# VladimirP1/rs-sync

Hardware: AMD Instinct MI355X
Metric: ray-residuals/sec (PreSync sweep + Sync iter), 4096 frames x 2048 tracks (higher is better)
Workload: dtype f32

## Files before the change

### rs-sync_amd/csrc/kernels/sync64.hpp

```cpp
#pragma once

#pragma clang fp contract(off)

namespace {



struct Loss64Params {
    Rays64 rays;
    const FrameRec* frames;
    const uint32_t* sel;
    uint32_t n_sel;
    const d4* coef;
    int n_knots;
    double fs;
    const int32_t* kd;
    const double* fd;
    uint32_t n_delays;
    const uint32_t* grp;
    uint32_t n_grp;
    const double* M;
    const double* k;
    double* part_loss;
    double* part_grad;
    uint32_t slot0;
    const uint32_t* slots;
    uint32_t win_cap;
    uint32_t win_compact;
    uint32_t nb_run;
};

constexpr int kLossBatch = 5;
constexpr int kLossBatchWide = 3;

template <int RPT, bool GRAD, bool SIMPLE, int CAP = 0>
__global__ __launch_bounds__(kBlock, 3) void loss64_kernel(Loss64Params p) {
    constexpr int NB = GRAD ? 1 : (CAP ? kLossBatch : (RPT == 0 ? 2 : kLossBatchWide));
    d4* s_loss_win;
    uint32_t win_cap;
    if constexpr (CAP != 0) {
        __shared__ d4 s_loss_win_static[NB * 4 * CAP];
        s_loss_win = s_loss_win_static;
        win_cap = CAP;
    } else {
        extern __shared__ d4 s_loss_win_dynamic[];
        s_loss_win = s_loss_win_dynamic;
        win_cap = p.win_cap;
    }
    __shared__ double s_red[NB][2][4];
    const uint32_t nb_run = (GRAD || CAP) ? (uint32_t)NB : (p.nb_run < (uint32_t)NB ? (p.nb_run ? p.nb_run : 1u) : (uint32_t)NB);
    const int tid = threadIdx.x, lane = tid & 63, wave = tid >> 6;
    const uint32_t sf = p.slots ? p.slots[blockIdx.x] : blockIdx.x + p.slot0;
    const uint32_t g = p.grp ? p.grp[sf] : 0u;
    {
        bool any = false;
        for (uint32_t b = 0; b < p.n_delays; ++b) {
            const double f = p.fd[b * p.n_grp + g];
            any = any || f == f;
        }
        if (!any) {
            for (uint32_t b = tid; b < p.n_delays; b += kBlock) {
                p.part_loss[(size_t)b * p.n_sel + sf] = 0.0;
                if (GRAD) p.part_grad[(size_t)b * p.n_sel + sf] = 0.0;
            }
            return;
        }
    }
    const uint32_t fi = p.sel[sf];
    const FrameRec fr = p.frames[fi];
    const uint32_t N = fr.n;
    const double Mx = SIMPLE ? 0.0 : p.M[3 * sf], My = SIMPLE ? 0.0 : p.M[3 * sf + 1], Mz = SIMPLE ? 0.0 : p.M[3 * sf + 2];
    const double kk = p.k[sf];
    const d3 Mv = d3{Mx, My, Mz};
    const double inv_s = rs::loss_inv_s(SIMPLE, kk, Mv);

    for (uint32_t b0 = 0; b0 < p.n_delays; b0 += nb_run) {
        Spline64 sp[NB];
        int base[NB];
        double fdv[NB];
        bool on[NB], any_on = false;
        int kdv[NB];
#pragma unroll
        for (int q = 0; q < NB; ++q) {
            const uint32_t b = b0 + q;
            on[q] = (uint32_t)q < nb_run && b < p.n_delays;
            kdv[q] = on[q] ? p.kd[b * p.n_grp + g] : 0;
            fdv[q] = on[q] ? p.fd[b * p.n_grp + g] : 0.0;
            if (fdv[q] != fdv[q]) on[q] = false;
            any_on = any_on || on[q];
        }
        if (!any_on) {
            if ((uint32_t)tid < nb_run && b0 + tid < p.n_delays) {
                p.part_loss[(size_t)(b0 + tid) * p.n_sel + sf] = 0.0;
                if (GRAD) p.part_grad[(size_t)(b0 + tid) * p.n_sel + sf] = 0.0;
            }
            continue;
        }
        __syncthreads();
// ... 144 lines not shown
    const int32_t* kd;
    const double* fd;
    const uint32_t* grp;
    double* M;
    double* k;
    unsigned long long* stats;
    uint32_t* per_frame;
    int reeval;
    int max_iters;
    int32_t* init_h;
    uint64_t seed;
    uint32_t stream_base, stream_stride;
    const uint32_t* win_stream;
    int simple_k;
    uint32_t slot0;
    const uint32_t* order;
    uint32_t* evals_out;
    double* scratch;
    uint32_t scratch_rows;
    uint32_t scratch0;
    uint32_t win_cap;
    uint32_t win_compact;
    uint32_t win_bytes;
};

#ifndef RSSYNC_K3_TIMING
#define RSSYNC_K3_TIMING 0
#endif
#if RSSYNC_K3_TIMING && RSSYNC_K2_COUNTERS
#define K3_T0() const long long k3t0__ = clock64()
#define K3_ACC(v) do { (v) += clock64() - k3t0__; } while (0)
#define K3_ADD(i, n) do { if (threadIdx.x == 0) { atomicAdd(&g_k2_counters[i], (unsigned long long)(clock64() - k3t0__)); if (n) atomicAdd(&g_k2_counters[n], 1ull); } } while (0)
#define K3_FLUSH(ev) do { if (threadIdx.x == 0) { atomicAdd(&g_k2_counters[10], (unsigned long long)(ev).t_eval); atomicAdd(&g_k2_counters[11], (unsigned long long)(ev).evals); } } while (0)
#else
#define K3_T0() do { } while (0)
#define K3_ACC(v) do { } while (0)
#define K3_ADD(i, n) do { } while (0)
#define K3_FLUSH(ev) do { } while (0)
#endif

constexpr int kInitNone = (int)0x80000000;
constexpr int kNB = rs::kLbfgsBasis;

template <int RPT, int NW, bool EMU4 = false>
struct MotionEval64 {
    static_assert(!EMU4 || (RPT == 0 && NW == 1), "the emulation reads its rows from global memory, one wave");
// ... 85 lines not shown
    __device__ __forceinline__ double& alpha(int i) { return s_alpha[i]; }
    __device__ __forceinline__ void store(int op, const double sv[3], const double yv[3]) {
        __syncthreads();
        if (threadIdx.x == 0) {
            for (int c = 0; c < 3; ++c) { s_S[op][c] = sv[c]; s_Y[op][c] = yv[c]; }
            s_inv_ys[op] = 1.0 / rs::dot3(yv, sv);
        }
        __syncthreads();
    }
};

__device__ __forceinline__ double clamp_k(double k) { return rs::clamp_k64(k); }

template <int NW>
struct MotionLds {
    double part[2][NW][4];
    double S[kNB][3], Y[kNB][3];
    double rho[kNB], alpha[kNB];
    double inv_ys[kNB];
    double red[NW];
};

template <int RPT, int NW, bool SC1 = false, bool EMU4 = false>
__device__ __forceinline__ void opt_motion64_body(const Motion64Params& p, uint32_t sf, MotionLds<NW>& lds, d4* s_win, double* mk_out = nullptr,
                                                  uint32_t scratch_entry = 0) {
    constexpr int kThreads = 64 * NW;
    double (*s_part)[NW][4] = lds.part;
    double (*s_S)[3] = lds.S;
    double (*s_Y)[3] = lds.Y;
    double* s_rho = lds.rho;
    double* s_alpha = lds.alpha;
    double* s_inv_ys = lds.inv_ys;
    double* s_red = lds.red;
    const int tid = threadIdx.x;
    const uint32_t fi = p.sel[sf];
    const FrameRec fr = p.frames[fi];
    const uint32_t N = fr.n;
    const uint32_t grp = p.grp ? p.grp[sf] : 0u;
    const int kd = ld_m<SC1>(&p.kd[grp]);
    const double fd = ld_m<SC1>(&p.fd[grp]);
    const int pend = p.init_h ? ld_m<SC1>(&p.init_h[sf]) : kInitNone;
    const double m_x = ld_m<SC1>(&p.M[3 * sf]), m_y = ld_m<SC1>(&p.M[3 * sf + 1]), m_z = ld_m<SC1>(&p.M[3 * sf + 2]);
    const double m_k = ld_m<SC1>(&p.k[sf]);
    if (fd != fd) {
        if (tid == 0 && p.evals_out) p.evals_out[sf] = 0;
        if (mk_out) { mk_out[0] = m_x; mk_out[1] = m_y; mk_out[2] = m_z; mk_out[3] = m_k; }
        return;
    }

    Spline64 sp;
    sp.g = p.coef;
    sp.n = p.n_knots;
    sp.cap = (int)p.win_cap;
    sp.compact = (int)p.win_compact;
    frame_window64(sp, s_win, fr, kd);
    __syncthreads();

    MotionEval64<RPT, NW, EMU4> ev;
    ev.part = s_part;
    ev.buf = 0;
    ev.evals = 0;
    const int base = fr.base_knot + kd;
    ev.gP = nullptr;
    ev.g_rows = 0;
    ev.rpt = RPT;
    if constexpr (RPT != 0) {
// ... 60 lines not shown
                const double pm = p.simple_k ? sqrt(rs::dot(Pj, Pj)) : rs::dot(Pj, Mv);
                ss = fma(pm, pm, ss);
            }
        }
        const double sw = wave_sum_f64(ss);
        if ((tid & 63) == 0) s_red[tid >> 6] = sw;
        __syncthreads();
        tot = s_red[0];
#pragma unroll
        for (int w = 1; w < NW; ++w) tot += s_red[w];
        }
        kk = clamp_k(100.0 / sqrt(tot));
        x[0] = Mv.x; x[1] = Mv.y; x[2] = Mv.z;
        if (tid == 0) {
            if (!p.simple_k) { st_m<SC1>(&p.M[3 * sf], x[0]); st_m<SC1>(&p.M[3 * sf + 1], x[1]); st_m<SC1>(&p.M[3 * sf + 2], x[2]); }
            st_m<SC1>(&p.k[sf], kk);
            if (p.init_h) st_m<SC1>(&p.init_h[sf], (int32_t)kInitNone);
        }
    } else {
        x[0] = m_x; x[1] = m_y; x[2] = m_z;
        kk = m_k;
    }
    if (mk_out) { mk_out[0] = x[0]; mk_out[1] = x[1]; mk_out[2] = x[2]; mk_out[3] = kk; }
    if (p.max_iters <= 0 || p.simple_k) return;
    ev.k2 = kk * kk;
    if constexpr (EMU4) {
        if ((size_t)N * 24u <= (size_t)p.win_bytes) {
            __syncthreads();
            __attribute__((address_space(3))) double* l = (__attribute__((address_space(3))) double*)reinterpret_cast<double*>(s_win);
            for (uint32_t row = tid; row < N; row += kThreads) {
                l[row] = ev.gP[row];
                l[N + row] = ev.gP[ev.g_rows + row];
                l[2 * N + row] = ev.gP[2 * (size_t)ev.g_rows + row];
            }
            __syncthreads();
            ev.lP = l;
            ev.n_lds = N;
        }
    }

    LbfgsHistLds hist{s_S, s_Y, s_inv_ys, s_rho, s_alpha};
    int best_not_last = 0;
    K3_T0();
    const int it = rs::lbfgs3(ev, hist, x, p.max_iters , p.reeval, &best_not_last);
    K3_ADD(12, 13);
    K3_FLUSH(ev);
    if (mk_out) { mk_out[0] = x[0]; mk_out[1] = x[1]; mk_out[2] = x[2]; }
    if (tid == 0) {
        st_m<SC1>(&p.M[3 * sf], x[0]); st_m<SC1>(&p.M[3 * sf + 1], x[1]); st_m<SC1>(&p.M[3 * sf + 2], x[2]);
        if (p.stats) {
            atomicAdd(&p.stats[0], (unsigned long long)it);
            atomicAdd(&p.stats[1], (unsigned long long)ev.evals);
            atomicAdd(&p.stats[2], (unsigned long long)best_not_last);
        }
        if (p.per_frame) {
            p.per_frame[2 * sf] = (uint32_t)it;
            p.per_frame[2 * sf + 1] = (uint32_t)ev.evals;
        }
        if (p.evals_out) p.evals_out[sf] = (uint32_t)ev.evals;
    }
}

template <int RPT, int NW>
__global__ __launch_bounds__(64 * NW, NW == 4 ? (RPT == 0 ? 2 : (RPT <= 8 ? 3 : (RPT <= 24 ? 2 : 1))) : (NW == 1 ? (RPT >= 8 ? 3 : 4) : 2)) void opt_motion64_kernel(Motion64Params p) {
    __shared__ MotionLds<NW> lds;
    extern __shared__ d4 s_motion_win[];
    opt_motion64_body<RPT, NW>(p, p.order ? p.order[blockIdx.x + p.slot0] : blockIdx.x + p.slot0, lds, s_motion_win, nullptr,
                               p.scratch0 + blockIdx.x);
}

__global__ __launch_bounds__(1024) void motion_order_kernel(const uint32_t* __restrict__ evals, const uint32_t* __restrict__ list,
                                                            uint32_t* __restrict__ order, uint32_t pos0, uint32_t count) {
    __shared__ uint32_t s_bin[256];
    for (uint32_t b = threadIdx.x; b < 256; b += blockDim.x) s_bin[b] = 0;
    __syncthreads();
    for (uint32_t i = threadIdx.x; i < count; i += blockDim.x) {
        const uint32_t e = evals[list[pos0 + i]];
        atomicAdd(&s_bin[e < 255u ? e : 255u], 1u);
    }
    __syncthreads();
    if (threadIdx.x == 0) {
        uint32_t at = 0;
        for (int b = 255; b >= 0; --b) {
            const uint32_t n = s_bin[b];
            s_bin[b] = at;
            at += n;
        }
    }
    __syncthreads();
    for (uint32_t i = threadIdx.x; i < count; i += blockDim.x) {
        const uint32_t s = list[pos0 + i];
        const uint32_t e = evals[s];
        const uint32_t pos = atomicAdd(&s_bin[e < 255u ? e : 255u], 1u);
        order[pos0 + pos] = s;
    }
}

struct Debug64Params {
    Rays64 rays;
    const FrameRec* frames;
    uint32_t fi;
    const d4* coef;
    int n_knots;
    double fs;
    int32_t kd;
    double fd;
    double* P;
    double* dP;
};

__global__ __launch_bounds__(kBlock) void debug_problem64_kernel(Debug64Params p) {
    __shared__ d4 s_win[4 * kWinMax];
    const FrameRec fr = p.frames[p.fi];
    Spline64 sp;
    sp.g = p.coef;
    sp.n = p.n_knots;
    sp.cap = kWinMax;
    sp.compact = 0;
// ... 31 lines not shown
```

### rs-sync_amd/csrc/kernels/syncloop.hpp

```cpp
#pragma once

namespace {

constexpr int kMaxBt = 10, kHalfBt = 5;

struct SyncWin {
    double d, v;
    double x0;
    double l1, g1;
    int active, conv, hit, iters;
    int phase;
    int nf;
    int hit_prev;
};

struct SyncLoopParams {
    SyncWin* win;
    uint32_t n_win;
    uint32_t win0, win1;
    const double* part;
    uint32_t n_sel, rows;
    const uint32_t* chunk_off;
    const uint32_t* win_chunk_off;
    double* chunk_tmp;
    uint32_t chunk_stride;
    int32_t* mo_kd; double* mo_fd;
    int32_t* lg_kd; double* lg_fd;
    int32_t* tr_kd; double* tr_fd;
    double fs;
    double ts[11];
    double c_armijo, delay_b, search_center, search_radius;
    int it, max_outer;
    int nf_fixed;
    int nf_floor;
    double* ext_sums;
    int* n_active;
    double* trace;
};


__device__ __forceinline__ void split64_dev(double delay, double fs, int32_t* kd, double* fd) {
#pragma clang fp contract(off)
    if (delay != delay) { *kd = 0; *fd = delay; return; }
    const double D = delay * fs;
    const double kClamp = (double)(1 << 29);
    if (!(fabs(D) <= 1.79769313486231570e308)) { *kd = 0; *fd = 0.0; return; }
    const double fl = floor(D);
    if (fl > kClamp) { *kd = 1 << 29; *fd = 0.0; return; }
    if (fl < -kClamp) { *kd = -(1 << 29); *fd = 0.0; return; }
    *kd = (int32_t)fl;
    *fd = D - fl;
}

constexpr uint32_t kStageDoubles = 2048;
__device__ __forceinline__ void window_sums(const SyncLoopParams& p, uint32_t w, double* s_tot, double* s_stage) {
    const uint32_t c0 = p.win_chunk_off[w], c1 = p.win_chunk_off[w + 1], nc = c1 - c0;
    const uint32_t j_lo = p.chunk_off[c0], j_hi = p.chunk_off[c1], span = j_hi - j_lo;
    double* tmp = p.chunk_tmp + (size_t)w * (2 * kMaxBt) * p.chunk_stride;
    const bool staged = p.rows * span <= kStageDoubles;
    if (staged) {
        for (uint32_t e = threadIdx.x; e < p.rows * span; e += blockDim.x)
            s_stage[e] = p.part[(size_t)(e / span) * p.n_sel + j_lo + e % span];
        __syncthreads();
    }
    for (uint32_t e = threadIdx.x; e < p.rows * nc; e += blockDim.x) {
        const uint32_t r = e / nc, c = c0 + e % nc;
        double acc = 0.0;
        uint32_t j = p.chunk_off[c];
        const uint32_t j1 = p.chunk_off[c + 1];
        if (staged) {
            const double* row = s_stage + (size_t)r * span - j_lo;
            for (; j + 8 <= j1; j += 8) {
                double v[8];
#pragma unroll
                for (int q = 0; q < 8; ++q) v[q] = row[j + q];
#pragma unroll
                for (int q = 0; q < 8; ++q) acc += v[q];
            }
            for (; j < j1; ++j) acc += row[j];
        } else {
            const double* row = p.part + (size_t)r * p.n_sel;
            const uint32_t cnt = j1 - j;
            if (cnt <= 64) {
                double v[64];
#pragma unroll
                for (int q = 0; q < 64; ++q) v[q] = (uint32_t)q < cnt ? row[j + q] : 0.0;
#pragma unroll
                for (int q = 0; q < 64; ++q)
                    if ((uint32_t)q < cnt) acc += v[q];
            } else {
                for (; j < j1; ++j) acc += row[j];
            }
        }
        tmp[(size_t)r * p.chunk_stride + (c - c0)] = acc;
    }
    __syncthreads();
    for (uint32_t r = threadIdx.x; r < p.rows; r += blockDim.x) {
        const double* t = tmp + (size_t)r * p.chunk_stride;
        double acc = 0.0;
        uint32_t c = 0;
        for (; c + 16 <= nc; c += 16) {
            double v[16];
#pragma unroll
            for (int q = 0; q < 16; ++q) v[q] = t[c + q];
#pragma unroll
            for (int q = 0; q < 16; ++q) acc += v[q];
        }
        for (; c < nc; ++c) acc += t[c];
        s_tot[r] = acc;
    }
    __syncthreads();
}

__global__ __launch_bounds__(64) void sync_begin_kernel(SyncLoopParams p) {
#pragma clang fp contract(off)
    const uint32_t w = p.win0 + blockIdx.x * 64 + threadIdx.x;
    if (w >= p.win1) return;
    SyncWin& s = p.win[w];
    s.x0 = s.active ? s.d - p.delay_b * s.v : __builtin_nan("");
    split64_dev(s.active ? s.d : __builtin_nan(""), p.fs, &p.mo_kd[w], &p.mo_fd[w]);
    split64_dev(s.x0, p.fs, &p.lg_kd[w], &p.lg_fd[w]);
}

__device__ __forceinline__ bool trial_wanted(const SyncWin& s, int i) {
    if (!s.active) return false;
    return s.phase == 0 ? i < s.nf : i >= s.nf;
}

__device__ __forceinline__ void grad_decide(const SyncLoopParams& p, SyncWin& s, double l1, double g1) {
#pragma clang fp contract(off)
    if (s.active && s.phase == 0) {
        s.l1 = l1;
        s.g1 = g1;
        s.hit = -1;
        if (s.iters == 0 && !p.nf_fixed) {
            int i = 0;
            while (i < kMaxBt - 1 && p.ts[i] * fabs(s.g1) >= 1e-3) ++i;
            const int want = i + 2;
            s.nf = want < kHalfBt ? kHalfBt : (want > kMaxBt ? kMaxBt : want);
        }
    }
}
__device__ __forceinline__ void trial_delays(const SyncLoopParams& p, const SyncWin& s, int32_t* tr_kd, double* tr_fd, size_t stride) {
#pragma clang fp contract(off)
    for (int i = 0; i < kMaxBt; ++i) {
        const double td = trial_wanted(s, i) ? s.x0 - p.ts[i] * s.g1 : __builtin_nan("");
        split64_dev(td, p.fs, &tr_kd[(size_t)i * stride], &tr_fd[(size_t)i * stride]);
    }
}

__global__ __launch_bounds__(kBlock) void sync_sums_kernel(SyncLoopParams p) {
#pragma clang fp contract(off)
    __shared__ double s_tot[2 * kMaxBt];
    __shared__ double s_stage[kStageDoubles];
    const uint32_t w = blockIdx.x + p.win0;
    window_sums(p, w, s_tot, s_stage);
    for (uint32_t r = threadIdx.x; r < p.rows; r += blockDim.x) p.ext_sums[(size_t)r * p.n_win + w] = s_tot[r];
}
__device__ __forceinline__ void decision_sums(const SyncLoopParams& p, uint32_t w, double* s_tot, double* s_stage) {
    if (p.ext_sums) {
        for (uint32_t r = threadIdx.x; r < p.rows; r += blockDim.x) s_tot[r] = p.ext_sums[(size_t)r * p.n_win + w];
        __syncthreads();
    } else {
        window_sums(p, w, s_tot, s_stage);
    }
}

__global__ __launch_bounds__(kBlock) void sync_grad_kernel(SyncLoopParams p) {
#pragma clang fp contract(off)
    __shared__ double s_tot[2 * kMaxBt];
    __shared__ double s_stage[kStageDoubles];
    const uint32_t w = blockIdx.x + p.win0;
    decision_sums(p, w, s_tot, s_stage);
    if (threadIdx.x != 0) return;
    SyncWin& s = p.win[w];
    grad_decide(p, s, s_tot[0], s_tot[1]);
    trial_delays(p, s, p.tr_kd + w, p.tr_fd + w, p.n_win);
}

__device__ __forceinline__ void armijo(const SyncLoopParams& p, SyncWin& s, const double* lt, int b0, int b1) {
#pragma clang fp contract(off)
    if (!s.active || s.hit >= 0) return;
    const double m = s.g1 * s.g1;
    for (int i = b0; i < b1; ++i) {
        if (s.l1 - lt[i] >= p.ts[i] * p.c_armijo * m) {
            s.hit = i;
            break;
        }
    }
}

__device__ __forceinline__ bool step_decide(const SyncLoopParams& p, SyncWin& s, const double* lt, double* rows, size_t row_stride) {
#pragma clang fp contract(off)
    bool step_now = false;
    if (s.active) {
        if (s.phase == 0) {
// ... 10 lines not shown
        const double t = s.hit >= 0 ? p.ts[s.hit] : p.ts[kMaxBt];
        const int trials = s.hit >= 0 ? s.hit + 1 : kMaxBt;
        const double step = -t * g;
        s.v = p.delay_b * s.v + step;
        s.d += s.v;
        const double step_size = fabs(step);
        double* row = rows + (size_t)s.iters * row_stride;
        row[0] = s.d; row[1] = step; row[2] = v; row[3] = g; row[4] = t; row[5] = (double)trials;
        s.iters += 1;
        s.phase = 0;
        const int last = s.hit >= 0 ? s.hit : kMaxBt - 1;
        const int want = (last > s.hit_prev ? last : s.hit_prev) + 1;
        s.hit_prev = last;
        s.nf = p.nf_fixed ? p.nf_fixed : (want < p.nf_floor ? p.nf_floor : (want > kMaxBt ? kMaxBt : want));
        if (step_size < 1e-4) s.conv++; else s.conv = 0;
        bool stop = s.conv > 5;
        if (!stop && fabs(s.d - p.search_center) > p.search_radius) stop = true;
        if (stop || s.iters == p.max_outer) s.active = 0;
    }
    s.x0 = s.active ? s.d - p.delay_b * s.v : __builtin_nan("");
    return step_now;
}

__global__ __launch_bounds__(kBlock) void sync_step_kernel(SyncLoopParams p) {
#pragma clang fp contract(off)
    __shared__ double s_tot[2 * kMaxBt];
    __shared__ double s_stage[kStageDoubles];
    const uint32_t w = blockIdx.x + p.win0;
    decision_sums(p, w, s_tot, s_stage);
    if (threadIdx.x != 0) return;
    SyncWin& s = p.win[w];
    step_decide(p, s, s_tot, p.trace + (size_t)w * 6, (size_t)p.n_win * 6);
    if (s.active) atomicAdd(&p.n_active[p.it], 1);
    const bool go = s.active && s.phase == 0;
    split64_dev(go ? s.d : __builtin_nan(""), p.fs, &p.mo_kd[w], &p.mo_fd[w]);
    split64_dev(go ? s.x0 : __builtin_nan(""), p.fs, &p.lg_kd[w], &p.lg_fd[w]);
}

}
```

### rs-sync_amd/csrc/rssync_kernels.hip

```cpp
#include <hip/hip_runtime.h>

#include <dlfcn.h>

#include <algorithm>
#include <cmath>
#include <cstdio>
#include <cstdlib>
#include <cstring>
#include <mutex>
#include <string>
#include <thread>
#include <vector>

#ifndef RSSYNC_TEST_VARIANTS
#define RSSYNC_TEST_VARIANTS 0
#endif

#include "../../include/rssync_hip.h"
#include "track_hip.h"
#include "rectify_hip.h"
#include "stabilize_hip.h"
#include "color_hip.h"
#include "device_math.hpp"
#include "sync_math.hpp"
// ... 604 lines not shown
                case 4: hipLaunchKernelGGL((lmeds_kernel<4, 0, 0, true, true>), dim3(grid), dim3(kBlock), 0, c->stream, p); break;
                case 8: hipLaunchKernelGGL((lmeds_kernel<8, 0, 0, true, true>), dim3(grid), dim3(kBlock), 0, c->stream, p); break;
                case 16: hipLaunchKernelGGL((lmeds_kernel<16, 0, 0, true, true>), dim3(grid), dim3(kBlock), 0, c->stream, p); break;
                case 24: allow_dynamic_lds(lmeds_kernel<24, 0, 0, true, true>, 0);
                         hipLaunchKernelGGL((lmeds_kernel<24, 0, 0, true, true>), dim3(grid), dim3(kBlock), 0, c->stream, p); break;
                case 32: allow_dynamic_lds(lmeds_kernel<16, 0, 0, true, true, kWideBlock>, 0);
                         hipLaunchKernelGGL((lmeds_kernel<16, 0, 0, true, true, kWideBlock>), dim3(grid), dim3(kWideBlock), 0, c->stream, p); break;
                default: return set_err(c, "lmeds (fp64 rows): unsupported rows-per-thread");
            }
        }
        RS_HIP(hipGetLastError());
    }
    return 0;
}

bool loss_fixed80(const rship_ctx* c, int k) {
    return c->cls_cap64[k] == (uint32_t)kWinMax && (class_span(c, k) + 1.f <= (float)kWinMax || c->force_general);
}
uint32_t loss_nb_run(const rship_ctx* c, int k) {
    return loss_fixed80(c, k) ? (uint32_t)kLossBatch : std::max(1u, std::min((uint32_t)kLossBatchWide, kLossWinBytes / (c->cls_cap64[k] * 128u)));
}

template <bool GRAD, bool SIMPLE>
int launch_loss64(rship_ctx* c, const Loss64Params& p_in, hipStream_t st = nullptr, uint32_t slot0 = 0, uint32_t count = 0) {
    if (!st) st = c->stream;
    ProfScope ps(c, GRAD ? RSHIP_K_LOSS_GRAD : RSHIP_K_LOSS);
    for (const ClassRange& r : class_ranges(c, slot0, count)) {
        Loss64Params p = p_in;
        const int k = r.k;
        p.slots = r.list;
        p.slot0 = r.list ? 0u : c->h_cls_slots[r.pos0];
        const uint32_t cap64 = cap64_of(c, k);
        p.win_cap = cap64;
        p.win_compact = compact_of(c, k) ? 1u : 0u;
        const bool fixed80 = !GRAD && loss_fixed80(c, k);
        p.nb_run = GRAD ? 1u : loss_nb_run(c, k);
        const size_t dyn = fixed80 ? 0 : (size_t)p.nb_run * cap64 * 128u, dyn_small = win64_bytes(c, k);
        if (k == 0 && !c->no_small_loss) {
            hipLaunchKernelGGL((loss64_small_kernel<GRAD, SIMPLE>), dim3(r.count), dim3(64), dyn_small, st, p);
            RS_HIP(hipGetLastError());
            continue;
        }
        const int rpt = k == 0 ? rpt_for(c->cls_max_n[0]) : class_rpt(c, k);
#define RS_LOSS_CASE(R)                                                                                                        \
    case R:                                                                                                                    \
        if constexpr (!GRAD) {                                                                                                 \
            if (fixed80) { hipLaunchKernelGGL((loss64_kernel<R, GRAD, SIMPLE, kWinMax>), dim3(r.count), dim3(kBlock), 0, st, p); break; } \
        }                                                                                                                      \
        hipLaunchKernelGGL((loss64_kernel<R, GRAD, SIMPLE, 0>), dim3(r.count), dim3(kBlock), dyn, st, p);                      \
        break;
        switch (rpt) {
            RS_LOSS_CASE(0)
            RS_LOSS_CASE(4)
            RS_LOSS_CASE(8)
            RS_LOSS_CASE(16)
            RS_LOSS_CASE(24)
            RS_LOSS_CASE(32)
            default: return set_err(c, "loss: unsupported rows-per-thread");
        }
#undef RS_LOSS_CASE
        RS_HIP(hipGetLastError());
    }
    return 0;
}

constexpr uint32_t kOrderMinSlots = 512;

int launch_motion64(rship_ctx* c, const Motion64Params& p_in, hipStream_t st = nullptr, uint32_t slot0 = 0, uint32_t count = 0) {
    if (!st) st = c->stream;
    ProfScope ps(c, RSHIP_K_MOTION);
    for (const ClassRange& r : class_ranges(c, slot0, count)) {
        Motion64Params p = p_in;
        const int k = r.k;
        p.slot0 = r.pos0;
        p.win_cap = cap64_of(c, k);
        p.win_compact = compact_of(c, k) ? 1u : 0u;
        const size_t dyn = win64_bytes(c, k);
        p.win_bytes = (uint32_t)dyn;
        const uint32_t cnt = r.count;
        if (k == 0) {
            const uint32_t n = c->cls_max_n[0];
            if (n <= 64) hipLaunchKernelGGL((opt_motion64_kernel<1, 1>), dim3(cnt), dim3(64), dyn, st, p);
            else if (n <= 128) hipLaunchKernelGGL((opt_motion64_kernel<2, 1>), dim3(cnt), dim3(64), dyn, st, p);
            else if (n <= 192) hipLaunchKernelGGL((opt_motion64_kernel<3, 1>), dim3(cnt), dim3(64), dyn, st, p);
            else if (n <= 256) hipLaunchKernelGGL((opt_motion64_kernel<4, 1>), dim3(cnt), dim3(64), dyn, st, p);
            else hipLaunchKernelGGL((opt_motion64_kernel<8, 1>), dim3(cnt), dim3(64), dyn, st, p);
        } else if (k == 1) hipLaunchKernelGGL((opt_motion64_kernel<4, 4>), dim3(cnt), dim3(256), dyn, st, p);
        else if (k == 2) hipLaunchKernelGGL((opt_motion64_kernel<8, 4>), dim3(cnt), dim3(256), dyn, st, p);
        else if (k == 3 && class_rpt(c, 3) == 16) hipLaunchKernelGGL((opt_motion64_kernel<16, 4>), dim3(cnt), dim3(256), dyn, st, p);
        else if (k == 3) hipLaunchKernelGGL((opt_motion64_kernel<24, 4>), dim3(cnt), dim3(256), dyn, st, p);
        else if (k == 4) hipLaunchKernelGGL((opt_motion64_kernel<32, 4>), dim3(cnt), dim3(256), dyn, st, p);
        else {
            if (!p.scratch || p.scratch_rows < c->cls_max_n[5]) return set_err(c, "motion: no scratch for frames of more than 8192 tracks");
            p.scratch0 = r.pos0 - c->cls_off[5];
            hipLaunchKernelGGL((opt_motion64_kernel<0, 4>), dim3(cnt), dim3(256), dyn, st, p);
        }
        RS_HIP(hipGetLastError());
        if (p.evals_out && p.order && c->mo_order.p && p.max_iters > 0 && !p.simple_k && cnt >= kOrderMinSlots) {
            hipLaunchKernelGGL(motion_order_kernel, dim3(1), dim3(1024), 0, st, (const uint32_t*)p.evals_out, (const uint32_t*)c->cls_slots.p,
                               (uint32_t*)c->mo_order.p, r.pos0, cnt);
            RS_HIP(hipGetLastError());
        }
    }
    return 0;
}

int launch_plan_sum(rship_ctx* c, const double* in, uint32_t rows, uint32_t cols, uint32_t slot = 0, uint32_t n_slots = 1) {
    if (!c->plan_wins) return set_err(c, "no reduction plan set");
    const size_t cs = (size_t)rows * (c->plan_chunks + 1), ws = (size_t)rows * c->plan_wins;
    if (n_slots > 1 && (c->chunk_out.cap < cs * n_slots * 8 || c->win_out.cap < ws * n_slots * 8)) return set_err(c, "plan sum: the batch's buffers were not sized");
    if (n_slots == 1 && (ensure(c, c->chunk_out, cs * 8) || ensure(c, c->win_out, ws * 8))) return 1;
    ProfScope ps(c, RSHIP_K_REDUCE);
    hipLaunchKernelGGL(plan_sum_kernel, dim3(rows * c->plan_wins), dim3(64), 0, c->stream, in, cols,
                       c->plan_has_idx ? (const uint32_t*)c->plan_idx.p : nullptr, (const uint32_t*)c->plan_chunk_off.p,
                       c->plan_chunks, (const uint32_t*)c->plan_win_off.p, c->plan_wins, (double*)c->chunk_out.p + cs * slot,
                       (double*)c->win_out.p + ws * slot);
    RS_HIP(hipGetLastError());
    return 0;
}

int queue_sums_to_host(rship_ctx* c, uint32_t rows, size_t at, size_t* off_chunk, size_t* end) {
// ... 1272 lines not shown
int rship_sync_run(rship_ctx* c, const double* d0, int max_outer, double search_center, double search_radius,
                   int simplified, double* d_out, int32_t* iters, double* trace) {
    const int rc = sync_run_body(c, d0, max_outer, search_center, search_radius, simplified, d_out, iters, trace);
    if (rc && c->rccl_comm) rccl_abort_comm(c);
    return rc;
}
static int sync_run_body(rship_ctx* c, const double* d0, int max_outer, double search_center, double search_radius,
                         int simplified, double* d_out, int32_t* iters, double* trace) {
    DeviceGuard dev_guard(c);
    const bool ranked = c->rccl_comm != nullptr || c->loop_xchg != nullptr;
    if (!c->n_knots) return set_err(c, "no gyro spline uploaded");
    if (!ranked && check_ready(c)) return 1;
    const uint32_t W = c->n_grp, ns = c->n_sel;
    if (c->plan_wins != W || c->plan_has_idx || c->plan_len != ns) return set_err(c, "sync_run: the plan must be the selection's groups");
    if (max_outer <= 0) return set_err(c, "sync_run: no iterations");
    if (c->h_grp_off.size() != (size_t)W + 1) return set_err(c, "sync_run: no selection");
    const uint32_t G = ranked ? 1u : loop_groups(c, W);
    rccl_allreduce_fn allreduce = nullptr;
    if (ranked && !c->loop_xchg && !(allreduce = (rccl_allreduce_fn)rccl_sym(c, "ncclAllReduce"))) return 1;
    std::vector<double> xbuf;
    c->loop_exchanges = 0;
    int nf_fixed = 0;
    if (const char* e = std::getenv("RSSYNC_LOOP_FIRST_TRIALS")) { const int v = atoi(e); if (v >= 1 && v <= kMaxBt) nf_fixed = v; }
    int nf_floor = (!ranked && c->max_n >= 1024u) ? 1 : kHalfBt;
    if (const char* e = std::getenv("RSSYNC_LOOP_TRIALS_FLOOR")) { const int v = atoi(e); if (v >= 1 && v <= kMaxBt) nf_floor = v; }
    const int max_launch = 2 * max_outer;
    size_t off = 0;
    auto take = [&](size_t bytes) { size_t o = off; off += (bytes + 255) / 256 * 256; return o; };
    const size_t o_win = take(W * sizeof(SyncWin));
    const size_t o_mokd = take(W * 4), o_mofd = take(W * 8), o_lgkd = take(W * 4), o_lgfd = take(W * 8);
    const size_t o_trkd = take((size_t)kMaxBt * W * 4), o_trfd = take((size_t)kMaxBt * W * 8);
    const size_t nact_stride = ((size_t)max_launch * 4 + 255) / 256 * 256;
    const size_t o_nact = take((size_t)G * nact_stride);
    const size_t o_trace = take((size_t)W * max_outer * 48);
    const size_t o_tmp = take((size_t)W * 2 * kMaxBt * (c->plan_max_chunks + 1) * 8);
    const size_t o_ext = take((size_t)2 * kMaxBt * W * 8);
    if (ensure(c, c->loop_state, off)) return 1;
    char* base = (char*)c->loop_state.p;
    if (ensure(c, c->part, (size_t)2 * kMaxBt * (ns + 1) * 8)) return 1;
    while (c->loop_streams.size() < G) {
        hipStream_t st = nullptr;
        RS_HIP(hipStreamCreateWithFlags(&st, hipStreamNonBlocking));
        c->loop_streams.push_back(st);
    }
    if (!c->loop_ready) RS_HIP(hipEventCreateWithFlags(&c->loop_ready, hipEventDisableTiming));

// ... 19 lines not shown
    lp.chunk_stride = c->plan_max_chunks + 1;
    lp.mo_kd = (int32_t*)(base + o_mokd); lp.mo_fd = (double*)(base + o_mofd);
    lp.lg_kd = (int32_t*)(base + o_lgkd); lp.lg_fd = (double*)(base + o_lgfd);
    lp.tr_kd = (int32_t*)(base + o_trkd); lp.tr_fd = (double*)(base + o_trfd);
    lp.fs = c->fs;
    {
        double t = 1e-3;
        for (int i = 0; i <= kMaxBt; ++i) { lp.ts[i] = t; t *= .1; }
    }
    lp.c_armijo = 2e-4;
    lp.delay_b = .3;
    lp.search_center = search_center;
    lp.search_radius = search_radius;
    lp.max_outer = max_outer;
    lp.nf_fixed = nf_fixed;
    lp.nf_floor = nf_floor;
    lp.trace = (double*)(base + o_trace);
    lp.ext_sums = ranked ? (double*)(base + o_ext) : nullptr;

    Motion64Params mp{};
    if (fill_motion(c, mp)) return 1;
    mp.kd = lp.mo_kd;
    mp.fd = lp.mo_fd;
    Loss64Params qp{};
    qp.rays = rays64_of(c);
    qp.frames = (const FrameRec*)c->frames.p;
    qp.sel = (const uint32_t*)c->sel.p;
    qp.n_sel = ns;
    qp.coef = (const d4*)c->coef64.p;
    qp.n_knots = (int)c->n_knots;
    qp.fs = c->fs;
    qp.grp = W > 1 ? (const uint32_t*)c->grp.p : nullptr;
    qp.n_grp = W;
    qp.M = (const double*)c->M.p;
    qp.k = (const double*)c->k.p;
    qp.part_loss = (double*)c->part.p;

    struct Group {
        uint32_t w0, w1, s0, s1;
        hipStream_t st;
        int* n_active;
        int* h_nact;
        int it = 0;
        bool done = false;
    };
    std::vector<Group> groups(G);
    if (ensure_pinned(c, (size_t)G * nact_stride + 64)) return 1;
    {
        uint32_t w = 0;
        for (uint32_t g = 0; g < G; ++g) {
            Group& gr = groups[g];
            gr.w0 = w;
            const uint64_t target = (uint64_t)ns * (g + 1) / G;
            while (w < W && (g + 1 == G || c->h_grp_off[w + 1] <= target || w == gr.w0)) ++w;
            if (g + 1 == G) w = W;
            gr.w1 = w;
            gr.s0 = c->h_grp_off[gr.w0];
            gr.s1 = c->h_grp_off[gr.w1];
            gr.st = G == 1 ? c->stream : c->loop_streams[g];
            gr.n_active = (int*)(base + o_nact + (size_t)g * nact_stride);
            gr.h_nact = (int*)((char*)c->pinned + (size_t)g * nact_stride);
            gr.done = gr.w1 == gr.w0;
        }
    }
    {
        std::vector<std::pair<uint32_t, uint32_t>> ranges;
        for (const Group& gr : groups)
            if (gr.s1 > gr.s0)
                for (const ClassRange& r : class_ranges(c, gr.s0, gr.s1 - gr.s0)) ranges.emplace_back(r.pos0, r.count);
        if (prepare_order(c, ranges)) return 1;
    }
    if (G > 1) {
        RS_HIP(hipEventRecord(c->loop_ready, c->stream));
        for (Group& gr : groups) RS_HIP(hipStreamWaitEvent(gr.st, c->loop_ready, 0));
    }
    auto enqueue_iteration = [&](Group& gr) -> int {
        SyncLoopParams l = lp;
        l.win0 = gr.w0; l.win1 = gr.w1;
        l.n_active = gr.n_active;
        l.it = gr.it;
        const uint32_t nw = gr.w1 - gr.w0, cnt = gr.s1 - gr.s0;
        const dim3 ctl_block(nw > 64 ? 64 : kBlock);
        Loss64Params q = qp;
        auto loss_launch = [&](bool grad) -> int {
            if (simplified) return grad ? launch_loss64<true, true>(c, q, gr.st, gr.s0, cnt) : launch_loss64<false, true>(c, q, gr.st, gr.s0, cnt);
            return grad ? launch_loss64<true, false>(c, q, gr.st, gr.s0, cnt) : launch_loss64<false, false>(c, q, gr.st, gr.s0, cnt);
        };
        if (gr.it == 0) {
            hipLaunchKernelGGL(sync_begin_kernel, dim3((nw + 63) / 64), dim3(64), 0, gr.st, l);
            RS_HIP(hipGetLastError());
        }
        if (!simplified && cnt) {
            if (launch_motion64(c, mp, gr.st, gr.s0, cnt)) return 1;
        }
        q.kd = l.lg_kd; q.fd = l.lg_fd; q.n_delays = 1;
        q.part_grad = q.part_loss + (size_t)ns;
        if (cnt && loss_launch(true)) return 1;
        l.rows = 2;
        auto exchange = [&](uint32_t rows) -> int {
            if (!ranked) return 0;
            hipLaunchKernelGGL(sync_sums_kernel, dim3(nw), ctl_block, 0, gr.st, l);
            RS_HIP(hipGetLastError());
            c->loop_exchanges += 1;
            if (c->loop_xchg) {
                xbuf.resize((size_t)rows * W);
                RS_HIP(hipMemcpyAsync(xbuf.data(), l.ext_sums, xbuf.size() * 8, hipMemcpyDeviceToHost, gr.st));
                RS_HIP(hipStreamSynchronize(gr.st));
                const int rc = c->loop_xchg(c->loop_xchg_user, xbuf.data(), xbuf.size());
                if (rc) return set_err(c, "sync_run: the loop's host exchange failed (" + std::to_string(rc) + ")");
                RS_HIP(hipMemcpyAsync(l.ext_sums, xbuf.data(), xbuf.size() * 8, hipMemcpyHostToDevice, gr.st));
                RS_HIP(hipStreamSynchronize(gr.st));
                return 0;
            }
            const int rc = allreduce(l.ext_sums, l.ext_sums, (size_t)rows * W,  8,  0, c->rccl_comm, gr.st);
            if (rc) return set_err(c, "rccl: ncclAllReduce failed (" + std::to_string(rc) + ")");
            return 0;
        };
        if (exchange(2)) return 1;
        {
            ProfScope ps(c, RSHIP_K_REDUCE);
            hipLaunchKernelGGL(sync_grad_kernel, dim3(nw), ctl_block, 0, gr.st, l);
        }
        q.kd = l.tr_kd; q.fd = l.tr_fd; q.n_delays = kMaxBt;
        q.part_grad = nullptr;
        l.rows = kMaxBt;
        if (cnt && loss_launch(false)) return 1;
        if (exchange(kMaxBt)) return 1;
        {
            ProfScope ps(c, RSHIP_K_REDUCE);
            hipLaunchKernelGGL(sync_step_kernel, dim3(nw), ctl_block, 0, gr.st, l);
        }
        RS_HIP(hipGetLastError());
        gr.it += 1;
        return 0;
    };

    const int kLook = 8;
    auto run_group = [&](Group& gr) -> int {
        DeviceGuard guard(c);
        while (!gr.done) {
            const int later = !ranked ? kLook / 2 : (c->loop_xchg ? 1 : 2);
            const int first = (ranked && c->loop_xchg) ? 1 : kLook;
            const int until = std::min(max_launch, gr.it + (gr.it == 0 ? first : later));
            while (gr.it < until)
                if (enqueue_iteration(gr)) return 1;
            RS_HIP(hipMemcpyAsync(gr.h_nact, gr.n_active, (size_t)gr.it * 4, hipMemcpyDeviceToHost, gr.st));
            RS_HIP(hipStreamSynchronize(gr.st));
            gr.done = gr.h_nact[gr.it - 1] == 0 || gr.it >= max_launch;
        }
        return 0;
    };
    {
        std::vector<std::thread> workers;
        std::vector<int> rc(G, 0);
// ... 1763 lines not shown
```

Before: 135.7 billion.

## Fuse loss-gradient into motion kernel and fold ordering into step kernel

For the size classes that qualify, the per-frame loss/gradient pass now runs at the end of the motion-optimization kernel, reusing its LDS window instead of needing a separate loss-grad launch. The motion-order histogram kernel is folded into the step kernel as extra blocks. The window-sum reductions also skip trial rows that are not wanted, and a wider 1024-thread control block is used for windows with long spans. Together these cut kernel launches and redundant reduction work, at the cost of more LDS and registers in the motion kernel plus extra complexity.

After: 137.0 billion (median of 6 runs). No clear change (+1.0%).

```diff
diff --git a/rs-sync_amd/csrc/kernels/sync64.hpp b/rs-sync_amd/csrc/kernels/sync64.hpp
--- a/rs-sync_amd/csrc/kernels/sync64.hpp
+++ b/rs-sync_amd/csrc/kernels/sync64.hpp
@@ -33,6 +33,44 @@
 constexpr int kLossBatch = 5;
 constexpr int kLossBatchWide = 3;
 
+template <int RPT, bool SIMPLE>
+__device__ __forceinline__ void loss_grad_rows64(const Rays64& rays, const d4* coef, int n_knots, uint32_t win_cap, uint32_t win_compact,
+                                                 d4* s_win, double (*s_red)[4], const FrameRec& fr, int kd, double fd, d3 Mv, double inv_s,
+                                                 double fs, double& L_out, double& G_out) {
+    const int tid = threadIdx.x, lane = tid & 63, wave = tid >> 6;
+    const uint32_t N = fr.n;
+    __syncthreads();
+    Spline64 sp;
+    sp.g = coef;
+    sp.n = n_knots;
+    sp.cap = (int)win_cap;
+    sp.compact = (int)win_compact;
+    frame_window64<0>(sp, s_win, fr, kd);
+    __syncthreads();
+    const int base = fr.base_knot + kd;
+    double L = 0.0, G = 0.0;
+    const int rpt = RPT ? RPT : (int)((N + kBlock - 1) / kBlock);
+#pragma unroll 1
+    for (int j = 0; j < rpt; ++j) {
+        const uint32_t row = j * kBlock + tid;
+        if (row < N) {
+            const size_t idx = (size_t)fr.off + row;
+            const double2 X = rays.q0[idx], Y = rays.q1[idx], Z = rays.q2[idx], T = rays.q3[idx];
+            d3 P, dP;
+            residual_row64_auto<true, 0>(sp, X, Y, Z, T, base, fd, P, dP);
+            rs::loss_row<true, SIMPLE>(P, dP, Mv, inv_s, L, G);
+        }
+    }
+    const double Lw = wave_sum_f64(L), Gw = wave_sum_f64(G);
+    if (lane == 0) {
+        s_red[0][wave] = Lw;
+        s_red[1][wave] = Gw;
+    }
+    __syncthreads();
+    L_out = s_red[0][0] + s_red[0][1] + s_red[0][2] + s_red[0][3];
+    G_out = (s_red[1][0] + s_red[1][1] + s_red[1][2] + s_red[1][3]) * fs;
+}
+
 template <int RPT, bool GRAD, bool SIMPLE, int CAP = 0>
 __global__ __launch_bounds__(kBlock, 3) void loss64_kernel(Loss64Params p) {
     constexpr int NB = GRAD ? 1 : (CAP ? kLossBatch : (RPT == 0 ? 2 : kLossBatchWide));
@@ -74,6 +112,21 @@
     const d3 Mv = d3{Mx, My, Mz};
     const double inv_s = rs::loss_inv_s(SIMPLE, kk, Mv);
 
+    if constexpr (GRAD) {
+        static_assert(CAP == 0, "the gradient kernel's window is in dynamic LDS");
+        for (uint32_t b = 0; b < p.n_delays; ++b) {
+            const double fdb = p.fd[b * p.n_grp + g];
+            double Lb = 0.0, Gb = 0.0;
+            if (fdb == fdb)
+                loss_grad_rows64<RPT, SIMPLE>(p.rays, p.coef, p.n_knots, win_cap, p.win_compact, s_loss_win, s_red[0], fr, p.kd[b * p.n_grp + g],
+                                              fdb, Mv, inv_s, p.fs, Lb, Gb);
+            if (tid == 0) {
+                p.part_loss[(size_t)b * p.n_sel + sf] = Lb;
+                p.part_grad[(size_t)b * p.n_sel + sf] = Gb;
+            }
+        }
+        return;
+    }
     for (uint32_t b0 = 0; b0 < p.n_delays; b0 += nb_run) {
         Spline64 sp[NB];
         int base[NB];
@@ -264,6 +317,11 @@
     uint32_t win_cap;
     uint32_t win_compact;
     uint32_t win_bytes;
+    const int32_t* lg_kd;
+    const double* lg_fd;
+    double* part_loss;
+    double* part_grad;
+    double fs;
 };
 
 #ifndef RSSYNC_K3_TIMING
@@ -395,8 +453,8 @@
 };
 
 template <int RPT, int NW, bool SC1 = false, bool EMU4 = false>
-__device__ __forceinline__ void opt_motion64_body(const Motion64Params& p, uint32_t sf, MotionLds<NW>& lds, d4* s_win, double* mk_out = nullptr,
-                                                  uint32_t scratch_entry = 0) {
+__device__ __forceinline__ void opt_motion64_core(const Motion64Params& p, uint32_t sf, MotionLds<NW>& lds, d4* s_win, double* mk_out,
+                                                  uint32_t scratch_entry, double* left) {
     constexpr int kThreads = 64 * NW;
     double (*s_part)[NW][4] = lds.part;
     double (*s_S)[3] = lds.S;
@@ -415,6 +473,7 @@
     const int pend = p.init_h ? ld_m<SC1>(&p.init_h[sf]) : kInitNone;
     const double m_x = ld_m<SC1>(&p.M[3 * sf]), m_y = ld_m<SC1>(&p.M[3 * sf + 1]), m_z = ld_m<SC1>(&p.M[3 * sf + 2]);
     const double m_k = ld_m<SC1>(&p.k[sf]);
+    left[0] = m_x; left[1] = m_y; left[2] = m_z; left[3] = m_k;
     if (fd != fd) {
         if (tid == 0 && p.evals_out) p.evals_out[sf] = 0;
         if (mk_out) { mk_out[0] = m_x; mk_out[1] = m_y; mk_out[2] = m_z; mk_out[3] = m_k; }
@@ -521,6 +580,8 @@
         kk = m_k;
     }
     if (mk_out) { mk_out[0] = x[0]; mk_out[1] = x[1]; mk_out[2] = x[2]; mk_out[3] = kk; }
+    left[3] = kk;
+    if (!p.simple_k) { left[0] = x[0]; left[1] = x[1]; left[2] = x[2]; }
     if (p.max_iters <= 0 || p.simple_k) return;
     ev.k2 = kk * kk;
     if constexpr (EMU4) {
@@ -558,6 +619,30 @@
         }
         if (p.evals_out) p.evals_out[sf] = (uint32_t)ev.evals;
     }
+    left[0] = x[0]; left[1] = x[1]; left[2] = x[2];
+}
+
+template <int RPT, int NW, bool SC1 = false, bool EMU4 = false>
+__device__ __forceinline__ void opt_motion64_body(const Motion64Params& p, uint32_t sf, MotionLds<NW>& lds, d4* s_win, double* mk_out = nullptr,
+                                                  uint32_t scratch_entry = 0) {
+    double left[4];
+    opt_motion64_core<RPT, NW, SC1, EMU4>(p, sf, lds, s_win, mk_out, scratch_entry, left);
+    if constexpr (RPT != 0 && NW == 4 && !SC1 && !EMU4) {
+        if (!p.lg_fd) return;
+        const uint32_t grp = p.grp ? p.grp[sf] : 0u;
+        const double lfd = p.lg_fd[grp];
+        double Lt = 0.0, Gt = 0.0;
+        if (lfd == lfd) {
+            const FrameRec fr = p.frames[p.sel[sf]];
+            const d3 Mv = d3{left[0], left[1], left[2]};
+            loss_grad_rows64<RPT, false>(p.rays, p.coef, p.n_knots, p.win_cap, p.win_compact, s_win, lds.part[0], fr, p.lg_kd[grp], lfd, Mv,
+                                         rs::loss_inv_s(false, left[3], Mv), p.fs, Lt, Gt);
+        }
+        if (threadIdx.x == 0) {
+            p.part_loss[sf] = Lt;
+            p.part_grad[sf] = Gt;
+        }
+    }
 }
 
 template <int RPT, int NW>
@@ -568,9 +653,8 @@
                                p.scratch0 + blockIdx.x);
 }
 
-__global__ __launch_bounds__(1024) void motion_order_kernel(const uint32_t* __restrict__ evals, const uint32_t* __restrict__ list,
-                                                            uint32_t* __restrict__ order, uint32_t pos0, uint32_t count) {
-    __shared__ uint32_t s_bin[256];
+__device__ __forceinline__ void motion_order_block(const uint32_t* __restrict__ evals, const uint32_t* __restrict__ list,
+                                                   uint32_t* __restrict__ order, uint32_t pos0, uint32_t count, uint32_t* s_bin) {
     for (uint32_t b = threadIdx.x; b < 256; b += blockDim.x) s_bin[b] = 0;
     __syncthreads();
     for (uint32_t i = threadIdx.x; i < count; i += blockDim.x) {
@@ -593,6 +677,11 @@
         const uint32_t pos = atomicAdd(&s_bin[e < 255u ? e : 255u], 1u);
         order[pos0 + pos] = s;
     }
+}
+__global__ __launch_bounds__(1024) void motion_order_kernel(const uint32_t* __restrict__ evals, const uint32_t* __restrict__ list,
+                                                            uint32_t* __restrict__ order, uint32_t pos0, uint32_t count) {
+    __shared__ uint32_t s_bin[256];
+    motion_order_block(evals, list, order, pos0, count, s_bin);
 }
 
 struct Debug64Params {
diff --git a/rs-sync_amd/csrc/kernels/syncloop.hpp b/rs-sync_amd/csrc/kernels/syncloop.hpp
--- a/rs-sync_amd/csrc/kernels/syncloop.hpp
+++ b/rs-sync_amd/csrc/kernels/syncloop.hpp
@@ -1,8 +1,18 @@
 #pragma once
 
+#ifndef RSSYNC_SUM_WANTED_ROWS
+#define RSSYNC_SUM_WANTED_ROWS 1
+#endif
+#ifndef RSSYNC_STEP_ORDER
+#define RSSYNC_STEP_ORDER 1
+#endif
+
 namespace {
 
 constexpr int kMaxBt = 10, kHalfBt = 5;
+constexpr int kWideCtl = 1024;
+constexpr uint32_t kWideCtlSlots = 1024;
+constexpr int kMaxOrderJobs = 6;
 
 struct SyncWin {
     double d, v;
@@ -36,6 +46,12 @@
     double* ext_sums;
     int* n_active;
     double* trace;
+    int rows_are_trials;
+    uint32_t n_order;
+    uint32_t order_pos0[kMaxOrderJobs], order_count[kMaxOrderJobs];
+    const uint32_t* order_evals;
+    const uint32_t* order_list;
+    uint32_t* order_out;
 };
 
 
@@ -52,19 +68,42 @@
     *fd = D - fl;
 }
 
+__device__ __forceinline__ bool trial_wanted(const SyncWin& s, int i) {
+    if (!s.active) return false;
+    return s.phase == 0 ? i < s.nf : i >= s.nf;
+}
+
 constexpr uint32_t kStageDoubles = 2048;
+template <bool WIDE>
 __device__ __forceinline__ void window_sums(const SyncLoopParams& p, uint32_t w, double* s_tot, double* s_stage) {
     const uint32_t c0 = p.win_chunk_off[w], c1 = p.win_chunk_off[w + 1], nc = c1 - c0;
     const uint32_t j_lo = p.chunk_off[c0], j_hi = p.chunk_off[c1], span = j_hi - j_lo;
     double* tmp = p.chunk_tmp + (size_t)w * (2 * kMaxBt) * p.chunk_stride;
+    uint32_t want = (1u << p.rows) - 1u;
+#if RSSYNC_SUM_WANTED_ROWS
+    if (p.rows_are_trials) {
+        const SyncWin s = p.win[w];
+        want = 0;
+        for (int i = 0; i < kMaxBt; ++i)
+            if (trial_wanted(s, i)) want |= 1u << i;
+    }
+#endif
+    const uint32_t n_want = (uint32_t)__popc(want);
     const bool staged = p.rows * span <= kStageDoubles;
     if (staged) {
         for (uint32_t e = threadIdx.x; e < p.rows * span; e += blockDim.x)
-            s_stage[e] = p.part[(size_t)(e / span) * p.n_sel + j_lo + e % span];
+            if (want >> (e / span) & 1u) s_stage[e] = p.part[(size_t)(e / span) * p.n_sel + j_lo + e % span];
         __syncthreads();
     }
-    for (uint32_t e = threadIdx.x; e < p.rows * nc; e += blockDim.x) {
-        const uint32_t r = e / nc, c = c0 + e % nc;
+    for (uint32_t e = threadIdx.x; e < n_want * nc; e += blockDim.x) {
+        uint32_t r = 0;
+        for (uint32_t left = e / nc, m = want;; ++r, m >>= 1) {
+            if (m & 1u) {
+                if (!left) break;
+                --left;
+            }
+        }
+        const uint32_t c = c0 + e % nc;
         double acc = 0.0;
         uint32_t j = p.chunk_off[c];
         const uint32_t j1 = p.chunk_off[c + 1];
@@ -82,12 +121,15 @@
             const double* row = p.part + (size_t)r * p.n_sel;
             const uint32_t cnt = j1 - j;
             if (cnt <= 64) {
-                double v[64];
-#pragma unroll
-                for (int q = 0; q < 64; ++q) v[q] = (uint32_t)q < cnt ? row[j + q] : 0.0;
-#pragma unroll
-                for (int q = 0; q < 64; ++q)
-                    if ((uint32_t)q < cnt) acc += v[q];
+                constexpr int kFly = WIDE ? 32 : 64;
+                for (uint32_t q0 = 0; q0 < cnt; q0 += kFly) {
+                    double v[kFly];
+#pragma unroll
+                    for (int q = 0; q < kFly; ++q) v[q] = q0 + q < cnt ? row[j + q0 + q] : 0.0;
+#pragma unroll
+                    for (int q = 0; q < kFly; ++q)
+                        if (q0 + q < cnt) acc += v[q];
+                }
             } else {
                 for (; j < j1; ++j) acc += row[j];
             }
@@ -99,14 +141,16 @@
         const double* t = tmp + (size_t)r * p.chunk_stride;
         double acc = 0.0;
         uint32_t c = 0;
-        for (; c + 16 <= nc; c += 16) {
-            double v[16];
-#pragma unroll
-            for (int q = 0; q < 16; ++q) v[q] = t[c + q];
-#pragma unroll
-            for (int q = 0; q < 16; ++q) acc += v[q];
-        }
-        for (; c < nc; ++c) acc += t[c];
+        if (want >> r & 1u) {
+            for (; c + 16 <= nc; c += 16) {
+                double v[16];
+#pragma unroll
+                for (int q = 0; q < 16; ++q) v[q] = t[c + q];
+#pragma unroll
+                for (int q = 0; q < 16; ++q) acc += v[q];
+            }
+            for (; c < nc; ++c) acc += t[c];
+        }
         s_tot[r] = acc;
     }
     __syncthreads();
@@ -120,11 +164,6 @@
     s.x0 = s.active ? s.d - p.delay_b * s.v : __builtin_nan("");
     split64_dev(s.active ? s.d : __builtin_nan(""), p.fs, &p.mo_kd[w], &p.mo_fd[w]);
     split64_dev(s.x0, p.fs, &p.lg_kd[w], &p.lg_fd[w]);
-}
-
-__device__ __forceinline__ bool trial_wanted(const SyncWin& s, int i) {
-    if (!s.active) return false;
-    return s.phase == 0 ? i < s.nf : i >= s.nf;
 }
 
 __device__ __forceinline__ void grad_decide(const SyncLoopParams& p, SyncWin& s, double l1, double g1) {
@@ -149,29 +188,32 @@
     }
 }
 
-__global__ __launch_bounds__(kBlock) void sync_sums_kernel(SyncLoopParams p) {
+template <int BLOCK>
+__global__ __launch_bounds__(BLOCK) void sync_sums_kernel(SyncLoopParams p) {
 #pragma clang fp contract(off)
     __shared__ double s_tot[2 * kMaxBt];
     __shared__ double s_stage[kStageDoubles];
     const uint32_t w = blockIdx.x + p.win0;
-    window_sums(p, w, s_tot, s_stage);
+    window_sums<(BLOCK > kBlock)>(p, w, s_tot, s_stage);
     for (uint32_t r = threadIdx.x; r < p.rows; r += blockDim.x) p.ext_sums[(size_t)r * p.n_win + w] = s_tot[r];
 }
+template <bool WIDE>
 __device__ __forceinline__ void decision_sums(const SyncLoopParams& p, uint32_t w, double* s_tot, double* s_stage) {
     if (p.ext_sums) {
         for (uint32_t r = threadIdx.x; r < p.rows; r += blockDim.x) s_tot[r] = p.ext_sums[(size_t)r * p.n_win + w];
         __syncthreads();
     } else {
-        window_sums(p, w, s_tot, s_stage);
-    }
-}
-
-__global__ __launch_bounds__(kBlock) void sync_grad_kernel(SyncLoopParams p) {
+        window_sums<WIDE>(p, w, s_tot, s_stage);
+    }
+}
+
+template <int BLOCK>
+__global__ __launch_bounds__(BLOCK) void sync_grad_kernel(SyncLoopParams p) {
 #pragma clang fp contract(off)
     __shared__ double s_tot[2 * kMaxBt];
     __shared__ double s_stage[kStageDoubles];
     const uint32_t w = blockIdx.x + p.win0;
-    decision_sums(p, w, s_tot, s_stage);
+    decision_sums<(BLOCK > kBlock)>(p, w, s_tot, s_stage);
     if (threadIdx.x != 0) return;
     SyncWin& s = p.win[w];
     grad_decide(p, s, s_tot[0], s_tot[1]);
@@ -228,12 +270,20 @@
     return step_now;
 }
 
-__global__ __launch_bounds__(kBlock) void sync_step_kernel(SyncLoopParams p) {
+template <int BLOCK>
+__global__ __launch_bounds__(BLOCK) void sync_step_kernel(SyncLoopParams p) {
 #pragma clang fp contract(off)
     __shared__ double s_tot[2 * kMaxBt];
     __shared__ double s_stage[kStageDoubles];
+#if RSSYNC_STEP_ORDER
+    if (blockIdx.x >= p.win1 - p.win0) {
+        const uint32_t j = blockIdx.x - (p.win1 - p.win0);
+        motion_order_block(p.order_evals, p.order_list, p.order_out, p.order_pos0[j], p.order_count[j], reinterpret_cast<uint32_t*>(s_stage));
+        return;
+    }
+#endif
     const uint32_t w = blockIdx.x + p.win0;
-    decision_sums(p, w, s_tot, s_stage);
+    decision_sums<(BLOCK > kBlock)>(p, w, s_tot, s_stage);
     if (threadIdx.x != 0) return;
     SyncWin& s = p.win[w];
     step_decide(p, s, s_tot, p.trace + (size_t)w * 6, (size_t)p.n_win * 6);
diff --git a/rs-sync_amd/csrc/rssync_kernels.hip b/rs-sync_amd/csrc/rssync_kernels.hip
--- a/rs-sync_amd/csrc/rssync_kernels.hip
+++ b/rs-sync_amd/csrc/rssync_kernels.hip
@@ -650,12 +650,13 @@
 }
 
 template <bool GRAD, bool SIMPLE>
-int launch_loss64(rship_ctx* c, const Loss64Params& p_in, hipStream_t st = nullptr, uint32_t slot0 = 0, uint32_t count = 0) {
+int launch_loss64(rship_ctx* c, const Loss64Params& p_in, hipStream_t st = nullptr, uint32_t slot0 = 0, uint32_t count = 0, uint32_t skip_classes = 0) {
     if (!st) st = c->stream;
     ProfScope ps(c, GRAD ? RSHIP_K_LOSS_GRAD : RSHIP_K_LOSS);
     for (const ClassRange& r : class_ranges(c, slot0, count)) {
         Loss64Params p = p_in;
         const int k = r.k;
+        if (skip_classes >> k & 1u) continue;
         p.slots = r.list;
         p.slot0 = r.list ? 0u : c->h_cls_slots[r.pos0];
         const uint32_t cap64 = cap64_of(c, k);
@@ -693,8 +694,10 @@
 }
 
 constexpr uint32_t kOrderMinSlots = 512;
-
-int launch_motion64(rship_ctx* c, const Motion64Params& p_in, hipStream_t st = nullptr, uint32_t slot0 = 0, uint32_t count = 0) {
+constexpr uint32_t kFusedGradClasses = 1u << 1 | 1u << 2 | 1u << 3 | 1u << 4;
+
+int launch_motion64(rship_ctx* c, const Motion64Params& p_in, hipStream_t st = nullptr, uint32_t slot0 = 0, uint32_t count = 0,
+                    std::vector<std::pair<uint32_t, uint32_t>>* order_later = nullptr) {
     if (!st) st = c->stream;
     ProfScope ps(c, RSHIP_K_MOTION);
     for (const ClassRange& r : class_ranges(c, slot0, count)) {
@@ -703,7 +706,7 @@
         p.slot0 = r.pos0;
         p.win_cap = cap64_of(c, k);
         p.win_compact = compact_of(c, k) ? 1u : 0u;
-        const size_t dyn = win64_bytes(c, k);
+        const size_t dyn = std::max(win64_bytes(c, k), (p.lg_fd && (kFusedGradClasses >> k & 1u)) ? (size_t)cap64_of(c, k) * 128u : (size_t)0);
         p.win_bytes = (uint32_t)dyn;
         const uint32_t cnt = r.count;
         if (k == 0) {
@@ -725,6 +728,7 @@
         }
         RS_HIP(hipGetLastError());
         if (p.evals_out && p.order && c->mo_order.p && p.max_iters > 0 && !p.simple_k && cnt >= kOrderMinSlots) {
+            if (order_later) { order_later->emplace_back(r.pos0, cnt); continue; }
             hipLaunchKernelGGL(motion_order_kernel, dim3(1), dim3(1024), 0, st, (const uint32_t*)p.evals_out, (const uint32_t*)c->cls_slots.p,
                                (uint32_t*)c->mo_order.p, r.pos0, cnt);
             RS_HIP(hipGetLastError());
@@ -2043,6 +2047,8 @@
     c->loop_exchanges = 0;
     int nf_fixed = 0;
     if (const char* e = std::getenv("RSSYNC_LOOP_FIRST_TRIALS")) { const int v = atoi(e); if (v >= 1 && v <= kMaxBt) nf_fixed = v; }
+    bool fused = true;
+    if (const char* e = std::getenv("RSSYNC_SYNC_FUSED")) fused = !(e[0] == '0' && !e[1]);
     int nf_floor = (!ranked && c->max_n >= 1024u) ? 1 : kHalfBt;
     if (const char* e = std::getenv("RSSYNC_LOOP_TRIALS_FLOOR")) { const int v = atoi(e); if (v >= 1 && v <= kMaxBt) nf_floor = v; }
     const int max_launch = 2 * max_outer;
@@ -2108,6 +2114,14 @@
     if (fill_motion(c, mp)) return 1;
     mp.kd = lp.mo_kd;
     mp.fd = lp.mo_fd;
+    const bool fuse_grad = fused && !simplified;
+    if (fuse_grad) {
+        mp.lg_kd = lp.lg_kd;
+        mp.lg_fd = lp.lg_fd;
+        mp.part_loss = (double*)c->part.p;
+        mp.part_grad = (double*)c->part.p + (size_t)ns;
+        mp.fs = c->fs;
+    }
     Loss64Params qp{};
     qp.rays = rays64_of(c);
     qp.frames = (const FrameRec*)c->frames.p;
@@ -2129,6 +2143,8 @@
         int* h_nact;
         int it = 0;
         bool done = false;
+        uint32_t max_span = 0;
+        bool grad_launch = true;
     };
     std::vector<Group> groups(G);
     if (ensure_pinned(c, (size_t)G * nact_stride + 64)) return 1;
@@ -2147,6 +2163,12 @@
             gr.n_active = (int*)(base + o_nact + (size_t)g * nact_stride);
             gr.h_nact = (int*)((char*)c->pinned + (size_t)g * nact_stride);
             gr.done = gr.w1 == gr.w0;
+            for (uint32_t v = gr.w0; v < gr.w1; ++v) gr.max_span = std::max(gr.max_span, c->h_grp_off[v + 1] - c->h_grp_off[v]);
+            if (fuse_grad && gr.s1 > gr.s0) {
+                gr.grad_launch = false;
+                for (const ClassRange& r : class_ranges(c, gr.s0, gr.s1 - gr.s0))
+                    if (!(kFusedGradClasses >> r.k & 1u)) gr.grad_launch = true;
+            }
         }
     }
     {
@@ -2166,26 +2188,32 @@
         l.n_active = gr.n_active;
         l.it = gr.it;
         const uint32_t nw = gr.w1 - gr.w0, cnt = gr.s1 - gr.s0;
-        const dim3 ctl_block(nw > 64 ? 64 : kBlock);
+        const bool wide_ctl = RSSYNC_SUM_WANTED_ROWS && gr.max_span > kWideCtlSlots;
+        const dim3 ctl_block(wide_ctl ? kWideCtl : (nw > 64 ? 64 : kBlock));
+#define RS_CTL_LAUNCH(K, GRID) do { if (wide_ctl) hipLaunchKernelGGL((K<kWideCtl>), dim3(GRID), ctl_block, 0, gr.st, l); \
+                                    else hipLaunchKernelGGL((K<kBlock>), dim3(GRID), ctl_block, 0, gr.st, l); } while (0)
+        std::vector<std::pair<uint32_t, uint32_t>> order_jobs;
+        const bool step_order = RSSYNC_STEP_ORDER && fused && ctl_block.x >= (uint32_t)kBlock;
         Loss64Params q = qp;
-        auto loss_launch = [&](bool grad) -> int {
+        auto loss_launch = [&](bool grad, uint32_t skip = 0u) -> int {
             if (simplified) return grad ? launch_loss64<true, true>(c, q, gr.st, gr.s0, cnt) : launch_loss64<false, true>(c, q, gr.st, gr.s0, cnt);
-            return grad ? launch_loss64<true, false>(c, q, gr.st, gr.s0, cnt) : launch_loss64<false, false>(c, q, gr.st, gr.s0, cnt);
+            return grad ? launch_loss64<true, false>(c, q, gr.st, gr.s0, cnt, skip) : launch_loss64<false, false>(c, q, gr.st, gr.s0, cnt);
         };
         if (gr.it == 0) {
             hipLaunchKernelGGL(sync_begin_kernel, dim3((nw + 63) / 64), dim3(64), 0, gr.st, l);
             RS_HIP(hipGetLastError());
         }
         if (!simplified && cnt) {
-            if (launch_motion64(c, mp, gr.st, gr.s0, cnt)) return 1;
+            if (launch_motion64(c, mp, gr.st, gr.s0, cnt, step_order ? &order_jobs : nullptr)) return 1;
         }
         q.kd = l.lg_kd; q.fd = l.lg_fd; q.n_delays = 1;
         q.part_grad = q.part_loss + (size_t)ns;
-        if (cnt && loss_launch(true)) return 1;
+        if (cnt && gr.grad_launch && loss_launch(true, fuse_grad ? kFusedGradClasses : 0u)) return 1;
         l.rows = 2;
+        l.rows_are_trials = 0;
         auto exchange = [&](uint32_t rows) -> int {
             if (!ranked) return 0;
-            hipLaunchKernelGGL(sync_sums_kernel, dim3(nw), ctl_block, 0, gr.st, l);
+            RS_CTL_LAUNCH(sync_sums_kernel, nw);
             RS_HIP(hipGetLastError());
             c->loop_exchanges += 1;
             if (c->loop_xchg) {
@@ -2205,17 +2233,25 @@
         if (exchange(2)) return 1;
         {
             ProfScope ps(c, RSHIP_K_REDUCE);
-            hipLaunchKernelGGL(sync_grad_kernel, dim3(nw), ctl_block, 0, gr.st, l);
+            RS_CTL_LAUNCH(sync_grad_kernel, nw);
         }
         q.kd = l.tr_kd; q.fd = l.tr_fd; q.n_delays = kMaxBt;
         q.part_grad = nullptr;
         l.rows = kMaxBt;
+        l.rows_are_trials = 1;
         if (cnt && loss_launch(false)) return 1;
         if (exchange(kMaxBt)) return 1;
+        if (order_jobs.size() > (size_t)kMaxOrderJobs) return set_err(c, "sync_run: more order segments than size classes");
+        l.n_order = (uint32_t)order_jobs.size();
+        for (uint32_t j = 0; j < l.n_order; ++j) { l.order_pos0[j] = order_jobs[j].first; l.order_count[j] = order_jobs[j].second; }
+        l.order_evals = (const uint32_t*)mp.evals_out;
+        l.order_list = (const uint32_t*)c->cls_slots.p;
+        l.order_out = (uint32_t*)c->mo_order.p;
         {
             ProfScope ps(c, RSHIP_K_REDUCE);
-            hipLaunchKernelGGL(sync_step_kernel, dim3(nw), ctl_block, 0, gr.st, l);
-        }
+            RS_CTL_LAUNCH(sync_step_kernel, nw + l.n_order);
+        }
+#undef RS_CTL_LAUNCH
         RS_HIP(hipGetLastError());
         gr.it += 1;
         return 0;
```
